# Sbte/RAILS

Hardware: AMD Instinct MI355X
Metric: RAILS iterations/sec (+ A*V SpMM HBM GB/s in roofline), m=1M rows/GPU, k=128, fp64 (higher is better)
Workload: dtype f64

## Files before the change

include/rails_hip.h:

```cpp
#ifndef RAILS_HIP_H
#define RAILS_HIP_H

#include <stddef.h>
#include <stdint.h>

#ifdef __cplusplus
extern "C" {
#endif

#define RAILS_OK 0
#define RAILS_EINVAL -1
#define RAILS_EHIP -2
#define RAILS_ENOMEM -3
#define RAILS_ELAPACK -4
#define RAILS_ECOMM -5
#define RAILS_ENODEV -6

typedef struct rails_ctx rails_ctx;
typedef struct rails_csr rails_csr;
typedef struct rails_panel rails_panel;

const char *rails_last_error(void);
const char *rails_version(void);

// ... 114 lines not shown
int rails_orthogonalize(rails_ctx *ctx, rails_panel *V, int k_old, int w, int method, int *used);
int rails_orthogonalize_deflated(rails_ctx *ctx, rails_panel *V, int k_old, int w, const rails_panel *N, int nc0, int q, int method, int *used);

int rails_resid_lanczos(rails_ctx *ctx, const rails_panel *AV, int avc0, const rails_panel *MV, int mvc0, int k,
                        const double *T_host, int ldt, const rails_panel *B, int bc0, int p, int L,
                        double *H_host, int ldh, int *steps);

int rails_lanczos_start(rails_ctx *ctx, const rails_panel *AV, int avc0, const rails_panel *MV, int mvc0, int k,
                        const rails_panel *B, int bc0, int p, double *sums_host);

int rails_lanczos_vectors(rails_ctx *ctx, const double *S_host, int lds, int w, rails_panel *Out, int oc0);
int rails_lanczos_release(rails_ctx *ctx);

int rails_ctx_reserve_staging(rails_ctx *ctx, size_t bytes);
int rails_timer_start(rails_ctx *ctx);
int rails_timer_stop(rails_ctx *ctx, double *ms);


void rails_sb03md(char dico, char job, char fact, char trans, int n, double *A, int lda, double *X, int ldx,
                  double *scale, int *info);
void rails_sb03md_counts(long *smith, long *schur);
void rails_sb03md_adi_counts(long *extended, long *fresh);
void rails_sb03md_set_pause(int calls);
void rails_dsyev(char jobz, char uplo, int n, double *a, int lda, double *w, int *info);
void rails_dsteqr(char compz, int n, double *d, double *e, double *z, int ldz, double *work, int *info);
void rails_dgemm(char transa, char transb, int m, int n, int k, double alpha, const double *A, int lda, const double *B,
                 int ldb, double beta, double *C, int ldc);
void rails_dtrsm(char side, char uplo, char transa, char diag, int m, int n, double alpha, const double *A, int lda, double *B, int ldb);
void rails_dpotrf(char uplo, int n, double *a, int lda, int *info);
void rails_dpstrf(char uplo, int n, double *a, int lda, int *piv, int *rank, double tol, int *info);
void rails_range_basis(int m, int n, double *a, int lda, double tol, double *q, int ldq, int *rank, int *info);
int rails_host_lapack_init(const char *path);
const char *rails_host_lapack_path(void);

#ifdef __cplusplus
}
#endif
#endif
```

rails_amd/_lib.py:

```python
import ctypes as C
import os

_HERE = os.path.dirname(os.path.abspath(__file__))
LIB_PATH = os.path.join(_HERE, "lib", "librails_hip.so")

_dp = C.POINTER(C.c_double)
_ip = C.POINTER(C.c_int)
_i64p = C.POINTER(C.c_int64)
_i32p = C.POINTER(C.c_int32)
_vp = C.c_void_p

ALLREDUCE_FN = C.CFUNCTYPE(C.c_int, C.c_void_p, C.c_void_p, C.c_size_t, C.c_void_p)
HALO_FN = C.CFUNCTYPE(C.c_int, C.c_void_p, C.c_void_p, C.c_void_p, C.c_int, C.c_void_p)
APPLY_FN = C.CFUNCTYPE(C.c_int, C.c_void_p, C.c_int, C.c_void_p, C.c_int, C.c_int, C.c_void_p, C.c_int)

SIGNATURES = {
    "rails_last_error": (C.c_char_p, []),
    "rails_version": (C.c_char_p, []),
    "rails_ctx_create": (C.c_int, [C.c_int, _vp, C.POINTER(_vp)]),
    "rails_ctx_destroy": (C.c_int, [_vp]),
    "rails_ctx_sync": (C.c_int, [_vp]),
    "rails_ctx_stream": (_vp, [_vp]),
    "rails_ctx_set_meter": (C.c_int, [_vp, C.c_int]),
    "rails_ctx_enable_library_gemm": (C.c_int, [_vp]),
# ... 55 lines not shown
    "rails_lu_solve": (C.c_int, [_vp, _vp, C.c_int, _vp, C.c_int, C.c_int, _vp, C.c_int]),
    "rails_lu_stats": (C.c_int, [_vp, _i64p, C.c_int]),
    "rails_csr_create_lu": (C.c_int, [_vp, _vp, C.POINTER(_vp)]),
    "rails_panel_random": (C.c_int, [_vp, _vp, C.c_int, C.c_int]),
    "rails_gram": (C.c_int, [_vp, _vp, C.c_int, C.c_int, _vp, C.c_int, C.c_int, _dp, C.c_int]),
    "rails_panel_gemm": (C.c_int, [_vp, C.c_double, _vp, C.c_int, C.c_int, _dp, C.c_int, C.c_int, C.c_double, _vp, C.c_int]),
    "rails_panel_gemm_wide": (C.c_int, [_vp, C.c_double, _vp, C.c_int, C.c_int, _dp, C.c_int, C.c_int, C.c_double, _vp, C.c_int]),
    "rails_orthogonalize": (C.c_int, [_vp, _vp, C.c_int, C.c_int, C.c_int, _ip]),
    "rails_orthogonalize_deflated": (C.c_int, [_vp, _vp, C.c_int, C.c_int, _vp, C.c_int, C.c_int, C.c_int, _ip]),
    "rails_resid_lanczos": (C.c_int, [_vp, _vp, C.c_int, _vp, C.c_int, C.c_int, _dp, C.c_int, _vp, C.c_int, C.c_int, C.c_int,
                                      _dp, C.c_int, _ip]),
    "rails_lanczos_start": (C.c_int, [_vp, _vp, C.c_int, _vp, C.c_int, C.c_int, _vp, C.c_int, C.c_int, _dp]),
    "rails_lanczos_vectors": (C.c_int, [_vp, _dp, C.c_int, C.c_int, _vp, C.c_int]),
    "rails_lanczos_release": (C.c_int, [_vp]),
    "rails_timer_start": (C.c_int, [_vp]),
    "rails_timer_stop": (C.c_int, [_vp, _dp]),
    "rails_sb03md": (None, [C.c_char, C.c_char, C.c_char, C.c_char, C.c_int, _dp, C.c_int, _dp, C.c_int, _dp, _ip]),
    "rails_dsyev": (None, [C.c_char, C.c_char, C.c_int, _dp, C.c_int, _dp, _ip]),
    "rails_dsteqr": (None, [C.c_char, C.c_int, _dp, _dp, _dp, C.c_int, _dp, _ip]),
    "rails_ctx_reserve_staging": (C.c_int, [_vp, C.c_size_t]),
    "rails_sb03md_set_pause": (None, [C.c_int]),
    "rails_sb03md_counts": (None, [C.POINTER(C.c_long), C.POINTER(C.c_long)]),
    "rails_sb03md_adi_counts": (None, [C.POINTER(C.c_long), C.POINTER(C.c_long)]),
    "rails_dtrsm": (None, [C.c_char, C.c_char, C.c_char, C.c_char, C.c_int, C.c_int, C.c_double, _dp, C.c_int, _dp, C.c_int]),
    "rails_dgemm": (None, [C.c_char, C.c_char, C.c_int, C.c_int, C.c_int, C.c_double, _dp, C.c_int, _dp, C.c_int, C.c_double, _dp, C.c_int]),
    "rails_dpotrf": (None, [C.c_char, C.c_int, _dp, C.c_int, _ip]),
    "rails_dpstrf": (None, [C.c_char, C.c_int, _dp, C.c_int, _ip, _ip, C.c_double, _ip]),
    "rails_range_basis": (None, [C.c_int, C.c_int, _dp, C.c_int, C.c_double, _dp, C.c_int, _ip, _ip]),
    "rails_host_lapack_init": (C.c_int, [C.c_char_p]),
    "rails_host_lapack_path": (C.c_char_p, []),
}

_lib = None


class RailsError(RuntimeError):
    pass


def load():
    global _lib
    if _lib is not None:
        return _lib
    if not os.path.exists(LIB_PATH):
        raise RailsError(
            "rails_amd: %s is missing -- build it with `python -c 'import __graft_entry__ as g; g.build()'` "
# ... 23 lines not shown
```

rails_amd/csrc/host_numerics.cpp:

```cpp
#include <dlfcn.h>

#include <algorithm>
#include <atomic>
#include <chrono>
#include <utility>
#include <cmath>
#include <cstdio>
#include <cstdlib>
#include <cstring>
#include <mutex>
#include <string>
#include <vector>

#include "rails_hip.h"

void rails_set_error(const char *fmt, ...);

namespace {

extern "C" {
typedef int (*lp_select2)(const double *, const double *);
typedef void (*lp_dsyev)(const char *, const char *, const int *, double *, const int *, double *, double *, const int *, int *);
typedef void (*lp_dsyevd)(const char *, const char *, const int *, double *, const int *, double *, double *, const int *, int *, const int *, int *);
typedef void (*lp_dsteqr)(const char *, const int *, double *, double *, double *, const int *, double *, int *);
// ... 327 lines not shown
    double wq = 0.0;
    int lwork = -1;
    g_lp.dgeqp3(&m, &n, a, &lda, jpvt.data(), tau.data(), &wq, &lwork, info);
    if (*info != 0) return;
    lwork = (int)wq + 1;
    std::vector<double> work((size_t)lwork);
    g_lp.dgeqp3(&m, &n, a, &lda, jpvt.data(), tau.data(), work.data(), &lwork, info);
    if (*info != 0) return;
    const double r11 = std::fabs(a[0]);
    int r = 0;
    while (r < kmin && std::fabs(a[r + (size_t)r * lda]) > tol * r11 && r11 > 0.0) ++r;
    *rank = r;
    if (r == 0) return;
    for (int j = 0; j < r; ++j)
        for (int i = 0; i < m; ++i) q[i + (size_t)j * ldq] = a[i + (size_t)j * lda];
    lwork = -1;
    g_lp.dorgqr(&m, &r, &r, q, &ldq, tau.data(), &wq, &lwork, info);
    if (*info != 0) return;
    lwork = (int)wq + 1;
    work.resize((size_t)lwork);
    g_lp.dorgqr(&m, &r, &r, q, &ldq, tau.data(), work.data(), &lwork, info);
}

static int &sb03md_smith_pause()
{
    static thread_local int pause = 0;
    return pause;
}
static int &sb03md_factored_pause()
{
    static thread_local int pause = 0;
    return pause;
}
extern "C" void rails_sb03md_set_pause(int calls) { sb03md_smith_pause() = sb03md_factored_pause() = calls > 0 ? calls : 0; }
static std::atomic<long> g_sb03md_smith{0}, g_sb03md_schur{0};
extern "C" void rails_sb03md_counts(long *smith, long *schur)
{
    if (smith) *smith = g_sb03md_smith.load();
    if (schur) *schur = g_sb03md_schur.load();
}

static bool smith_lyapunov(bool tr, int n, const double *A, int lda, double *X, int ldx)
{
    if (!g_lp.dgetrf || !g_lp.dgetrs) return false;
    const size_t nn = (size_t)n * n;
    std::vector<double> M(nn), S(nn), Ak(nn), Y(nn), T1(nn), T2(nn), C(nn);
    double trace = 0.0;
    for (int j = 0; j < n; ++j) {
        for (int i = 0; i < n; ++i) {
            M[i + (size_t)j * n] = tr ? A[i + (size_t)j * lda] : A[j + (size_t)i * lda];
            C[i + (size_t)j * n] = 0.5 * (X[i + (size_t)j * ldx] + X[j + (size_t)i * ldx]);
        }
        trace += A[j + (size_t)j * lda];
    }
    const double p = -trace / n;
    if (!(p > 0.0) || !std::isfinite(p)) return false;
    S = M;
// ... 34 lines not shown
    }
    if (!converged) return false;
    for (int j = 0; j < n; ++j)
        for (int i = 0; i < j; ++i) {
            const double v = 0.5 * (Y[i + (size_t)j * n] + Y[j + (size_t)i * n]);
            Y[i + (size_t)j * n] = v;
            Y[j + (size_t)i * n] = v;
        }
    gemm('N', 'N', n, n, n, M.data(), n, Y.data(), n, T1.data(), n);
    double r2 = 0.0;
    for (int j = 0; j < n; ++j)
        for (int i = 0; i < n; ++i) {
            const double r = T1[i + (size_t)j * n] + T1[j + (size_t)i * n] - C[i + (size_t)j * n];
            r2 += r * r;
        }
    if (!(std::sqrt(r2) <= 2e-15 * (2.0 * fro(M) * fro(Y) + fro(C)))) return false;
    for (int j = 0; j < n; ++j)
        for (int i = 0; i < n; ++i) X[i + (size_t)j * ldx] = Y[i + (size_t)j * n];
    return true;
}

struct AdiCache {
    int n = 0, L = 0;
    bool tr = false;
    double a = 0.0, b = 0.0;
    std::vector<double> M, shift;
    std::vector<std::vector<double>> LUs;
    std::vector<std::vector<int>> ips;
    std::vector<std::vector<double>> Inv;
};
static AdiCache &adi_cache()
{
    static thread_local AdiCache c;
    return c;
}
static std::atomic<long> g_adi_extended{0}, g_adi_fresh{0};
extern "C" void rails_sb03md_adi_counts(long *extended, long *fresh)
{
    if (extended) *extended = g_adi_extended.load();
    if (fresh) *fresh = g_adi_fresh.load();
}

static bool extend_lu(int n1, int n, const std::vector<double> &LU1, const std::vector<int> &ip1, std::vector<double> &S, std::vector<int> &ip)
{
    const int nb = n - n1, one = 1;
    const double d_one = 1.0, d_mone = -1.0;
// ... 45 lines not shown
        S = J1;
        return true;
    }
    const double d_one = 1.0, d_mone = -1.0, d_zero = 0.0;
    double *A12 = &S[(size_t)n1 * n], *A21 = &S[n1], *A22 = &S[n1 + (size_t)n1 * n];
    std::vector<double> E((size_t)n1 * nb), F((size_t)nb * n1), Cm((size_t)nb * nb), G((size_t)nb * n1);
    g_lp.dgemm("N", "N", &n1, &nb, &n1, &d_one, J1.data(), &n1, A12, &n, &d_zero, E.data(), &n1);
    g_lp.dgemm("N", "N", &nb, &n1, &n1, &d_one, A21, &n, J1.data(), &n1, &d_zero, F.data(), &nb);
    for (int j = 0; j < nb; ++j)
        for (int i = 0; i < nb; ++i) Cm[i + (size_t)j * nb] = A22[i + (size_t)j * n];
    g_lp.dgemm("N", "N", &nb, &nb, &n1, &d_mone, A21, &n, E.data(), &n1, &d_one, Cm.data(), &nb);
    if (!invert_dense(nb, Cm)) return false;
    g_lp.dgemm("N", "N", &nb, &n1, &nb, &d_one, Cm.data(), &nb, F.data(), &nb, &d_zero, G.data(), &nb);
    for (int j = 0; j < n1; ++j) memcpy(&S[(size_t)j * n], &J1[(size_t)j * n1], sizeof(double) * n1);
    g_lp.dgemm("N", "N", &n1, &n1, &nb, &d_one, E.data(), &n1, G.data(), &nb, &d_one, S.data(), &n);
    g_lp.dgemm("N", "N", &n1, &nb, &nb, &d_mone, E.data(), &n1, Cm.data(), &nb, &d_zero, A12, &n);
    for (int j = 0; j < n1; ++j)
        for (int i = 0; i < nb; ++i) A21[i + (size_t)j * n] = -G[i + (size_t)j * nb];
    for (int j = 0; j < nb; ++j)
        for (int i = 0; i < nb; ++i) A22[i + (size_t)j * n] = Cm[i + (size_t)j * nb];
    return true;
}

static bool adi_lyapunov_lowrank_once(bool tr, int n, const double *A, int lda, double *X, int ldx, bool *not_applicable, bool from_scratch, bool *inherited)
{
    *inherited = false;
    *not_applicable = false;
    if (!g_lp.dgetrf || !g_lp.dgetrs) return false;
    static const bool trace_lr = getenv("RAILS_SB03MD_TRACE") != nullptr;
    auto now = [] { return std::chrono::duration<double, std::milli>(std::chrono::steady_clock::now().time_since_epoch()).count(); };
    const double t_begin = now();
    double t_mark = t_begin, t_factor = 0, t_bounds = 0, t_lu = 0, t_terms = 0, t_form = 0;
    auto lap = [&](double &acc) {
        const double t = now();
        acc += t - t_mark;
        t_mark = t;
    };
    const size_t nn = (size_t)n * n;
    std::vector<double> C(nn), W(nn);
    double trc = 0.0, dmax = 0.0;
    for (int j = 0; j < n; ++j) {
        for (int i = 0; i < n; ++i) C[i + (size_t)j * n] = 0.5 * (X[i + (size_t)j * ldx] + X[j + (size_t)i * ldx]);
        trc += C[j + (size_t)j * n];
        dmax = std::max(dmax, std::fabs(C[j + (size_t)j * n]));
    }
    if (!(dmax > 0.0) || !std::isfinite(dmax)) return false;
    const double sign = trc >= 0.0 ? 1.0 : -1.0;
    for (size_t q = 0; q < nn; ++q) W[q] = sign * C[q];
    std::vector<int> piv(n);
    int rank = 0, info = 0;
    rails_dpstrf('U', n, W.data(), n, piv.data(), &rank, 1e-15 * dmax, &info);
    if (info < 0 || rank <= 0 || rank > n / 3) {
        *not_applicable = true;
        return false;
    }
    std::vector<double> F((size_t)n * rank, 0.0);
    for (int j = 0; j < n; ++j)
        for (int i = 0; i < rank && i <= j; ++i) F[piv[j] + (size_t)i * n] = W[i + (size_t)j * n];
    std::vector<double> M(nn);
    for (int j = 0; j < n; ++j)
        for (int i = 0; i < n; ++i) M[i + (size_t)j * n] = tr ? A[i + (size_t)j * lda] : A[j + (size_t)i * lda];
    lap(t_factor);
    const char N = 'N';
    const int one = 1;
    static const bool allow_inherit = !(getenv("RAILS_SB03MD_ADI_INHERIT") && atoi(getenv("RAILS_SB03MD_ADI_INHERIT")) == 0);
    AdiCache &cache = adi_cache();
    static const bool allow_explicit = !(getenv("RAILS_SB03MD_ADI_INVERSE") && atoi(getenv("RAILS_SB03MD_ADI_INVERSE")) == 0);
    const bool explicit_steps = allow_explicit && n >= 64;
    bool inherit = allow_inherit && !from_scratch && g_lp.dlaswp && g_lp.dtrsm && cache.n >= 32 && cache.tr == tr && n >= cache.n && n - cache.n <= 64 && cache.L >= 1 &&
                   (explicit_steps ? (int)cache.Inv.size() == cache.L : (int)cache.LUs.size() == cache.L);
    for (int j = 0; inherit && j < cache.n; ++j) inherit = memcmp(&M[(size_t)j * n], &cache.M[(size_t)j * cache.n], sizeof(double) * cache.n) == 0;
    double a = 0.0, b = 0.0;
    int L = 1;
    std::vector<double> shift;
    std::vector<std::vector<double>> LUs, Inv;
    std::vector<std::vector<int>> ips;
    std::vector<double> v(n), u(n);
    auto nrm = [&](std::vector<double> const &z) {
        double s2 = 0.0;
        for (int i = 0; i < n; ++i) s2 += z[i] * z[i];
        return std::sqrt(s2);
    };
    auto extent = [&](const std::vector<double> &LUp, const std::vector<int> &ipp, const std::vector<double> *InvP, double pshift, double *a_out, double *b_out) {
        for (int i = 0; i < n; ++i) v[i] = 1.0 + 0.37 * std::sin(1.0 + 2.3 * i);
        double bmax = 0.0, amin = 0.0;
        for (int it = 0; it < 6; ++it) {
            const double nv = nrm(v);
            for (int i = 0; i < n; ++i) v[i] /= nv;
            gemm('N', 'N', n, 1, n, M.data(), n, v.data(), n, u.data(), n);
            bmax = std::max(bmax, nrm(u));
            v = u;
        }
        for (int i = 0; i < n; ++i) v[i] = 1.0 + 0.37 * std::sin(1.0 + 2.3 * i);
        for (int it = 0; it < 6; ++it) {
            const double nv = nrm(v);
            for (int i = 0; i < n; ++i) v[i] /= nv;
            if (InvP) {
                gemm('N', 'N', n, 1, n, InvP->data(), n, v.data(), n, u.data(), n);
                v = u;
            } else {
                int inf = 0;
                g_lp.dgetrs(&N, &n, &one, LUp.data(), &n, ipp.data(), v.data(), &n, &inf);
                if (inf != 0) return false;
            }
            amin = nrm(v);
        }
        if (!(amin > 0.0) || !(bmax > 0.0) || !std::isfinite(amin) || !std::isfinite(bmax)) return false;
        const double lmin = 1.0 / amin - pshift;
        if (!(lmin > 0.0)) return false;
        *a_out = 0.8 * lmin, *b_out = 1.2 * bmax;
        if (!(*a_out < *b_out)) *a_out = 0.5 * *b_out;
        return true;
    };
    if (inherit) {
        a = cache.a, b = cache.b, L = cache.L, shift = cache.shift;
        LUs.assign(explicit_steps ? 0 : L, std::vector<double>());
        ips.assign(explicit_steps ? 0 : L, std::vector<int>());
        Inv.assign(explicit_steps ? L : 0, std::vector<double>());
        for (int i = 0; i < L && inherit; ++i) {
            std::vector<double> &S = explicit_steps ? Inv[i] : LUs[i];
            S = M;
            for (int j = 0; j < n; ++j) S[j + (size_t)j * n] -= shift[i];
            inherit = explicit_steps ? extend_inverse(cache.n, n, cache.Inv[i], S) : extend_lu(cache.n, n, cache.LUs[i], cache.ips[i], S, ips[i]);
        }
        lap(t_lu);
        double a_now = 0.0, b_now = 0.0;
        if (inherit && !((explicit_steps ? extent(Inv[0], std::vector<int>(), &Inv[0], shift[0], &a_now, &b_now) : extent(LUs[0], ips[0], nullptr, shift[0], &a_now, &b_now)) &&
                         a_now >= 0.8 * a && b_now <= 1.15 * b))
            inherit = false;
        lap(t_bounds);
    }
    if (!inherit) {
    std::vector<double> LU0 = M;
    std::vector<int> ip0(n);
    g_lp.dgetrf(&n, &n, LU0.data(), &n, ip0.data(), &info);
    if (info != 0) return false;
    if (!extent(LU0, ip0, nullptr, 0.0, &a, &b)) return false;
    lap(t_bounds);
    if (b / a > 1e5) return false;
    const double kappa = b / a, pi = 3.14159265358979323846;
    double best_cost = 1e300;
    for (int cand = 1; cand <= 8; cand *= 2) {
        double rho = cand == 1 ? (std::sqrt(kappa) - 1.0) / (std::sqrt(kappa) + 1.0) : std::min(0.999, 4.0 * std::exp(-pi * pi * cand / std::log(4.0 * kappa)));
        double sweeps = std::ceil(std::log(3e-9) / std::log(std::max(rho, 1e-300)));
        double cost = 4.0 * cand + cand * std::max(1.0, sweeps);
        if (cost < best_cost) best_cost = cost, L = cand;
    }
    shift.assign(1, std::sqrt(a * b));
    {
        std::vector<std::pair<double, double>> iv(1, std::make_pair(a, b));
        for (int l = L; l > 1; l /= 2) iv.push_back(std::make_pair(std::sqrt(iv.back().first * iv.back().second), 0.5 * (iv.back().first + iv.back().second)));
        shift.assign(1, std::sqrt(iv.back().first * iv.back().second));
        for (int lev = (int)iv.size() - 2; lev >= 0; --lev) {
            const double ab = iv[lev].first * iv[lev].second;
            std::vector<double> up;
            for (double x : shift) {
                const double d = std::sqrt(std::max(0.0, x * x - ab));
                up.push_back(x + d);
                up.push_back(x - d);
            }
            shift.swap(up);
        }
        std::sort(shift.begin(), shift.end());
    }
    LUs.assign(explicit_steps ? 0 : L, std::vector<double>());
    ips.assign(explicit_steps ? 0 : L, std::vector<int>(n));
    Inv.assign(explicit_steps ? L : 0, std::vector<double>());
    for (int i = 0; i < L; ++i) {
        std::vector<double> &S = explicit_steps ? Inv[i] : LUs[i];
        S = M;
        for (int j = 0; j < n; ++j) S[j + (size_t)j * n] -= shift[i];
        if (explicit_steps) {
            if (!invert_dense(n, S)) return false;
        } else {
            g_lp.dgetrf(&n, &n, S.data(), &n, ips[i].data(), &info);
            if (info != 0) return false;
        }
    }
    lap(t_lu);
    }
    (inherit ? g_adi_extended : g_adi_fresh)++;
    *inherited = inherit;
    lap(t_lu);
    const size_t blk = (size_t)n * rank;
    const int max_terms = std::max(64, 16 * L), max_cols = 8 * n;
    std::vector<double> Z, T(blk);
    Z.reserve(blk * 24);
    auto norm2 = [&](const double *z) {
        double s2 = 0.0;
        for (size_t q = 0; q < blk; ++q) s2 += z[q] * z[q];
        return s2;
    };
    std::vector<std::vector<double>> Sm(explicit_steps ? L : 0);
    for (int i = 0; i < (int)Sm.size(); ++i) {
        const double pj = shift[i], pp = shift[(i + L - 1) % L];
        const double f = std::sqrt(pj / pp), fg = f * (pj + pp);
        Sm[i].resize(nn);
        for (size_t q = 0; q < nn; ++q) Sm[i][q] = fg * Inv[i][q];
        for (int j = 0; j < n; ++j) Sm[i][j + (size_t)j * n] += f;
    }
    if (explicit_steps)
        gemm('N', 'N', n, rank, n, Inv[0].data(), n, F.data(), n, T.data(), n);
    else {
        T = F;
        g_lp.dgetrs(&N, &n, &rank, LUs[0].data(), &n, ips[0].data(), T.data(), &n, &info);
        if (info != 0) return false;
    }
    {
        const double f = std::sqrt(2.0 * shift[0]);
        for (size_t q = 0; q < blk; ++q) T[q] *= f;
    }
    Z.insert(Z.end(), T.begin(), T.end());
    double total = norm2(T.data()), cycle_start = total;
    bool converged = false;
    for (int j = 1; j < max_terms; ++j) {
        const int cur = j % L, prv = (j - 1) % L;
        const double pj = shift[cur], pp = shift[prv];
        const double *zp = Z.data() + (size_t)(j - 1) * blk;
        if (explicit_steps)
            gemm('N', 'N', n, rank, n, Sm[cur].data(), n, zp, n, T.data(), n);
        else {
            std::copy(zp, zp + blk, T.begin());
            g_lp.dgetrs(&N, &n, &rank, LUs[cur].data(), &n, ips[cur].data(), T.data(), &n, &info);
            if (info != 0) return false;
            const double f = std::sqrt(pj / pp), g = pj + pp;
            for (size_t q = 0; q < blk; ++q) T[q] = f * (zp[q] + g * T[q]);
        }
        const double n2 = norm2(T.data());
        if (!std::isfinite(n2) || n2 > 1e4 * total) return false;
        if ((int)((size_t)(j + 1) * rank) > max_cols) return false;
        Z.insert(Z.end(), T.begin(), T.end());
        total += n2;
        if (n2 <= 1e-17 * total) {
            converged = true;
            break;
        }
        if (cur == L - 1) {
            if (j >= 2 * L - 1 && n2 > 0.2 * cycle_start) {
                if (trace_lr) fprintf(stderr, "sb03md ADI: n %d, spectrum ~[%.3g, %.3g], %d shifts: term %d is %.2e of the same term one cycle earlier -- giving up\n", n, a, b, L, j, n2 / cycle_start);
                return false;
            }
            cycle_start = n2;
        }
    }
    lap(t_terms);
    if (trace_lr) fprintf(stderr, "sb03md ADI: n %d rank %d, spectrum ~[%.3g, %.3g], %d shifts, %d terms, converged %d\n", n, rank, a, b, L, (int)(Z.size() / blk), (int)converged);
    if (!converged) return false;
    const int cols = (int)(Z.size() / n);
    std::vector<double> Y(nn);
    if (g_lp.dsyrk) {
        const double one_d = 1.0, zero_d = 0.0;
        g_lp.dsyrk("U", "N", &n, &cols, &one_d, Z.data(), &n, &zero_d, Y.data(), &n);
        for (int j = 0; j < n; ++j)
            for (int i = 0; i < j; ++i) Y[j + (size_t)i * n] = Y[i + (size_t)j * n];
    } else {
        gemm('N', 'T', n, n, cols, Z.data(), n, Z.data(), n, Y.data(), n);
        for (int j = 0; j < n; ++j)
            for (int i = 0; i < j; ++i) {
                const double vv = 0.5 * (Y[i + (size_t)j * n] + Y[j + (size_t)i * n]);
                Y[i + (size_t)j * n] = vv;
                Y[j + (size_t)i * n] = vv;
            }
    }
    for (size_t q = 0; q < nn; ++q) Y[q] *= -sign;
    gemm('N', 'N', n, n, n, M.data(), n, Y.data(), n, W.data(), n);
    double r2 = 0.0, m2 = 0.0, y2 = 0.0, c2 = 0.0;
    for (int j = 0; j < n; ++j)
        for (int i = 0; i < n; ++i) {
            const double r = W[i + (size_t)j * n] + W[j + (size_t)i * n] - C[i + (size_t)j * n];
            r2 += r * r;
            m2 += M[i + (size_t)j * n] * M[i + (size_t)j * n];
            y2 += Y[i + (size_t)j * n] * Y[i + (size_t)j * n];
            c2 += C[i + (size_t)j * n] * C[i + (size_t)j * n];
        }
    lap(t_form);
    if (trace_lr)
        fprintf(stderr, "sb03md ADI: residual %.2e of %.2e allowed; ms: factor C %.2f, bounds %.2f, %d LU %.2f, terms %.2f, X = ZZ' + check %.2f, total %.2f\n", std::sqrt(r2),
                2e-15 * (2.0 * std::sqrt(m2 * y2) + std::sqrt(c2)), t_factor, t_bounds, L, t_lu, t_terms, t_form, now() - t_begin);
    if (!(std::sqrt(r2) <= 2e-15 * (2.0 * std::sqrt(m2 * y2) + std::sqrt(c2)))) return false;
    for (int j = 0; j < n; ++j)
        for (int i = 0; i < n; ++i) X[i + (size_t)j * ldx] = Y[i + (size_t)j * n];
    cache.n = n, cache.L = L, cache.tr = tr, cache.a = a, cache.b = b;
    cache.M.swap(M);
    cache.shift.swap(shift);
    cache.LUs.swap(LUs);
    cache.ips.swap(ips);
    cache.Inv.swap(Inv);
    return true;
}

static bool adi_lyapunov_lowrank(bool tr, int n, const double *A, int lda, double *X, int ldx, bool *not_applicable)
{
    bool inherited = false;
    if (adi_lyapunov_lowrank_once(tr, n, A, lda, X, ldx, not_applicable, false, &inherited)) return true;
    if (!inherited || *not_applicable) return false;
    return adi_lyapunov_lowrank_once(tr, n, A, lda, X, ldx, not_applicable, true, &inherited);
}

extern "C" void rails_sb03md(char dico, char job, char fact, char trans, int n, double *A, int lda, double *X, int ldx, double *scale,
                             int *info)
{
    *info = 0;
    if (n < 1) {
        fprintf(stderr, "rails_sb03md: n < 1 is not supported\n");
        return;
    }
    if ((dico != 'C' && dico != 'c') || (job != 'X' && job != 'x') || (fact != 'N' && fact != 'n')) {
        fprintf(stderr, "rails_sb03md: only DICO='C', JOB='X', FACT='N' is supported\n");
        *info = -1;
        return;
    }
    if (rails_host_lapack_init(nullptr) != RAILS_OK) {
        *info = -100;
        return;
    }
    if (!all_finite(n, n, A, lda) || !all_finite(n, n, X, ldx)) {
        fprintf(stderr, "rails_sb03md: A or C holds NaN or Inf entries\n");
        *info = n + 2;
        return;
    }
    const bool tr = (trans == 'T' || trans == 't' || trans == 'C' || trans == 'c');
    static const bool use_symmetric = [] {
        const char *e = getenv("RAILS_SB03MD_SYMMETRIC");
        return e ? atoi(e) != 0 : true;
    }();
    if (use_symmetric && n >= 8) {
        double amax = 0.0, asym = 0.0;
        for (int j = 0; j < n; ++j)
            for (int i = 0; i < j; ++i) {
                const double a = A[i + (size_t)j * lda], b = A[j + (size_t)i * lda];
                amax = std::max(amax, std::max(std::fabs(a), std::fabs(b)));
                asym = std::max(asym, std::fabs(a - b));
            }
        for (int i = 0; i < n; ++i) amax = std::max(amax, std::fabs(A[i + (size_t)i * lda]));
        if (amax > 0.0 && asym <= 1e-13 * amax) {
            std::vector<double> Q((size_t)n * n), lam(n), F((size_t)n * n), W((size_t)n * n);
            for (int j = 0; j < n; ++j)
                for (int i = 0; i < n; ++i) Q[i + (size_t)j * n] = 0.5 * (A[i + (size_t)j * lda] + A[j + (size_t)i * lda]);
            int sinfo = 0;
            if (g_lp.dsyevd) {
                int lwork = -1, liwork = -1, iq = 0;
                double wq = 0.0;
                g_lp.dsyevd("V", "U", &n, Q.data(), &n, lam.data(), &wq, &lwork, &iq, &liwork, &sinfo);
                lwork = (int)wq + 1;
// ... 8 lines not shown
            }
            if (sinfo == 0) {
                gemm('T', 'N', n, n, n, Q.data(), n, X, ldx, W.data(), n);
                gemm('N', 'N', n, n, n, W.data(), n, Q.data(), n, F.data(), n);
                bool singular = false;
                for (int j = 0; j < n && !singular; ++j)
                    for (int i = 0; i < n; ++i) {
                        const double den = lam[i] + lam[j];
                        if (!(std::fabs(den) > 1e-300)) {
                            singular = true;
                            break;
                        }
                        F[i + (size_t)j * n] /= den;
                    }
                if (!singular) {
                    gemm('N', 'N', n, n, n, Q.data(), n, F.data(), n, W.data(), n);
                    gemm('N', 'T', n, n, n, W.data(), n, Q.data(), n, F.data(), n);
                    for (int j = 0; j < n; ++j)
                        for (int i = 0; i < n; ++i) {
                            X[i + (size_t)j * ldx] = F[i + (size_t)j * n];
                            A[i + (size_t)j * lda] = (i == j) ? lam[i] : 0.0;
                        }
                    *scale = 1.0;
                    return;
                }
            }
        }
    }
    static const bool use_smith = [] {
        const char *e = getenv("RAILS_SB03MD_SMITH");
        return e ? atoi(e) != 0 : true;
    }();
    int &smith_pause = sb03md_smith_pause();
    int &lowrank_pause = sb03md_factored_pause();
    bool adi_na = false;
    if (use_smith && n >= 32) {
        if (smith_pause > 0)
            --smith_pause;
        else if ((lowrank_pause > 0 ? (--lowrank_pause, false) : (adi_lyapunov_lowrank(tr, n, A, lda, X, ldx, &adi_na) || (lowrank_pause = adi_na ? 0 : 30, false))) ||
                 smith_lyapunov(tr, n, A, lda, X, ldx)) {
            g_sb03md_smith++;
            *scale = 1.0;
            return;
        } else
            smith_pause = 30;
    }
    g_sb03md_schur++;
    std::vector<double> U((size_t)n * n), wr(n), wi(n), F((size_t)n * n), W((size_t)n * n);
    int sdim = 0, lwork = -1, linfo = 0;
    double wq = 0.0;
    g_lp.dgees("V", "N", nullptr, &n, A, &lda, &sdim, wr.data(), wi.data(), U.data(), &n, &wq, &lwork, nullptr, &linfo);
    lwork = std::max((int)wq, 3 * n);
    std::vector<double> work((size_t)lwork);
    g_lp.dgees("V", "N", nullptr, &n, A, &lda, &sdim, wr.data(), wi.data(), U.data(), &n, work.data(), &lwork, nullptr, &linfo);
    if (linfo != 0) {
        *info = linfo > n ? n : linfo;
        return;
    }
    gemm('T', 'N', n, n, n, U.data(), n, X, ldx, W.data(), n);
    gemm('N', 'N', n, n, n, W.data(), n, U.data(), n, F.data(), n);
    int isgn = 1, tinfo = 0;
    static const bool use_blocked = [] {
        const char *e = getenv("RAILS_SB03MD_BLOCKED");
        return e ? atoi(e) != 0 : true;
    }();
    bool done = false;
    if (g_lp.dtrsyl3 && use_blocked && n >= 64) {
        int liwork = -1, ldswork = -1, iq = 0, qinfo = 0;
        double sq[2] = {0.0, 0.0};
// ... 20 lines not shown
```

Before: 225.3.

## Restructure Lyapunov ADI solver with staged inheritance, reshifting, and adaptive backoff

Reworks the host-side low-rank ADI Lyapunov solver into a staged loop: inherited shifts, then re-shifting from freshly measured spectral bounds, then a from-scratch setup. An inherited attempt gives up early once it exceeds the previous call's term count. The fixed 30-call pause after failure becomes an exponential backoff capped at 32, and the ADI cache is cleared when the solver falls back. It also adds a per-call ring-buffer log of route, terms and time. The aim is to cut wasted ADI and Schur work in the small dense Lyapunov solves done each RAILS iteration, at the cost of more complex control flow and a small logging overhead on every call.

After: 221.2. -1.8%, worse.

```diff
diff --git a/include/rails_hip.h b/include/rails_hip.h
--- a/include/rails_hip.h
+++ b/include/rails_hip.h
@@ -160,6 +160,14 @@
 void rails_sb03md_counts(long *smith, long *schur);
 void rails_sb03md_adi_counts(long *extended, long *fresh);
 void rails_sb03md_set_pause(int calls);
+#define RAILS_SB03MD_ROUTE_SYMMETRIC 1
+#define RAILS_SB03MD_ROUTE_ADI_INHERITED 2
+#define RAILS_SB03MD_ROUTE_ADI_RESHIFTED 3
+#define RAILS_SB03MD_ROUTE_ADI_SCRATCH 4
+#define RAILS_SB03MD_ROUTE_SMITH 5
+#define RAILS_SB03MD_ROUTE_SCHUR 6
+int rails_sb03md_call_log(int max, int *n, int *route, int *terms, int *repeated, double *ms);
+void rails_sb03md_call_log_clear(void);
 void rails_dsyev(char jobz, char uplo, int n, double *a, int lda, double *w, int *info);
 void rails_dsteqr(char compz, int n, double *d, double *e, double *z, int ldz, double *work, int *info);
 void rails_dgemm(char transa, char transb, int m, int n, int k, double alpha, const double *A, int lda, const double *B,
diff --git a/rails_amd/_lib.py b/rails_amd/_lib.py
--- a/rails_amd/_lib.py
+++ b/rails_amd/_lib.py
@@ -101,6 +101,8 @@
     "rails_sb03md_set_pause": (None, [C.c_int]),
     "rails_sb03md_counts": (None, [C.POINTER(C.c_long), C.POINTER(C.c_long)]),
     "rails_sb03md_adi_counts": (None, [C.POINTER(C.c_long), C.POINTER(C.c_long)]),
+    "rails_sb03md_call_log": (C.c_int, [C.c_int, _ip, _ip, _ip, _ip, _dp]),
+    "rails_sb03md_call_log_clear": (None, []),
     "rails_dtrsm": (None, [C.c_char, C.c_char, C.c_char, C.c_char, C.c_int, C.c_int, C.c_double, _dp, C.c_int, _dp, C.c_int]),
     "rails_dgemm": (None, [C.c_char, C.c_char, C.c_int, C.c_int, C.c_int, C.c_double, _dp, C.c_int, _dp, C.c_int, C.c_double, _dp, C.c_int]),
     "rails_dpotrf": (None, [C.c_char, C.c_int, _dp, C.c_int, _ip]),
diff --git a/rails_amd/csrc/host_numerics.cpp b/rails_amd/csrc/host_numerics.cpp
--- a/rails_amd/csrc/host_numerics.cpp
+++ b/rails_amd/csrc/host_numerics.cpp
@@ -373,17 +373,66 @@
     g_lp.dorgqr(&m, &r, &r, q, &ldq, tau.data(), work.data(), &lwork, info);
 }
 
-static int &sb03md_smith_pause()
-{
-    static thread_local int pause = 0;
-    return pause;
-}
-static int &sb03md_factored_pause()
-{
-    static thread_local int pause = 0;
-    return pause;
-}
-extern "C" void rails_sb03md_set_pause(int calls) { sb03md_smith_pause() = sb03md_factored_pause() = calls > 0 ? calls : 0; }
+struct Sb03mdRest {
+    int rest = 0;
+    int pause = 0;
+    bool resting()
+    {
+        if (rest <= 0) return false;
+        --rest;
+        return true;
+    }
+    void failed() { rest = pause = pause > 0 ? std::min(2 * pause, 32) : 1; }
+    void succeeded() { pause = 0; }
+};
+static Sb03mdRest &sb03md_iterative_rest()
+{
+    static thread_local Sb03mdRest r;
+    return r;
+}
+static Sb03mdRest &sb03md_factored_rest()
+{
+    static thread_local Sb03mdRest r;
+    return r;
+}
+extern "C" void rails_sb03md_set_pause(int calls)
+{
+    Sb03mdRest forced;
+    forced.rest = calls > 0 ? calls : 0;
+    sb03md_iterative_rest() = sb03md_factored_rest() = forced;
+}
+
+struct Sb03mdCall {
+    int n, route, terms, repeated;
+    double ms;
+};
+struct Sb03mdLog {
+    static const int size = 256;
+    Sb03mdCall ring[size];
+    long count = 0;
+};
+static Sb03mdLog &sb03md_log()
+{
+    static thread_local Sb03mdLog log;
+    return log;
+}
+static double sb03md_now_ms() { return std::chrono::duration<double, std::milli>(std::chrono::steady_clock::now().time_since_epoch()).count(); }
+extern "C" int rails_sb03md_call_log(int max, int *n, int *route, int *terms, int *repeated, double *ms)
+{
+    const Sb03mdLog &log = sb03md_log();
+    const long held = std::min<long>(log.count, Sb03mdLog::size);
+    const int out = (int)std::min<long>(held, max > 0 ? max : 0);
+    for (int i = 0; i < out; ++i) {
+        const Sb03mdCall &c = log.ring[(log.count - out + i) % Sb03mdLog::size];
+        if (n) n[i] = c.n;
+        if (route) route[i] = c.route;
+        if (terms) terms[i] = c.terms;
+        if (repeated) repeated[i] = c.repeated;
+        if (ms) ms[i] = c.ms;
+    }
+    return out;
+}
+extern "C" void rails_sb03md_call_log_clear(void) { sb03md_log().count = 0; }
 static std::atomic<long> g_sb03md_smith{0}, g_sb03md_schur{0};
 extern "C" void rails_sb03md_counts(long *smith, long *schur)
 {
@@ -464,6 +513,7 @@
 
 struct AdiCache {
     int n = 0, L = 0;
+    int terms = 0;
     bool tr = false;
     double a = 0.0, b = 0.0;
     std::vector<double> M, shift;
@@ -555,17 +605,21 @@
     return true;
 }
 
-static bool adi_lyapunov_lowrank_once(bool tr, int n, const double *A, int lda, double *X, int ldx, bool *not_applicable, bool from_scratch, bool *inherited)
-{
-    *inherited = false;
+struct AdiOutcome {
+    int route = 0;
+    int terms = 0;
+    int wasted = 0;
+};
+
+static bool adi_lyapunov_lowrank(bool tr, int n, const double *A, int lda, double *X, int ldx, bool *not_applicable, AdiOutcome *outcome)
+{
     *not_applicable = false;
     if (!g_lp.dgetrf || !g_lp.dgetrs) return false;
     static const bool trace_lr = getenv("RAILS_SB03MD_TRACE") != nullptr;
-    auto now = [] { return std::chrono::duration<double, std::milli>(std::chrono::steady_clock::now().time_since_epoch()).count(); };
-    const double t_begin = now();
+    const double t_begin = sb03md_now_ms();
     double t_mark = t_begin, t_factor = 0, t_bounds = 0, t_lu = 0, t_terms = 0, t_form = 0;
     auto lap = [&](double &acc) {
-        const double t = now();
+        const double t = sb03md_now_ms();
         acc += t - t_mark;
         t_mark = t;
     };
@@ -600,7 +654,7 @@
     AdiCache &cache = adi_cache();
     static const bool allow_explicit = !(getenv("RAILS_SB03MD_ADI_INVERSE") && atoi(getenv("RAILS_SB03MD_ADI_INVERSE")) == 0);
     const bool explicit_steps = allow_explicit && n >= 64;
-    bool inherit = allow_inherit && !from_scratch && g_lp.dlaswp && g_lp.dtrsm && cache.n >= 32 && cache.tr == tr && n >= cache.n && n - cache.n <= 64 && cache.L >= 1 &&
+    bool inherit = allow_inherit && g_lp.dlaswp && g_lp.dtrsm && cache.n >= 32 && cache.tr == tr && n >= cache.n && n - cache.n <= 64 && cache.L >= 1 &&
                    (explicit_steps ? (int)cache.Inv.size() == cache.L : (int)cache.LUs.size() == cache.L);
     for (int j = 0; inherit && j < cache.n; ++j) inherit = memcmp(&M[(size_t)j * n], &cache.M[(size_t)j * cache.n], sizeof(double) * cache.n) == 0;
     double a = 0.0, b = 0.0;
@@ -614,10 +668,10 @@
         for (int i = 0; i < n; ++i) s2 += z[i] * z[i];
         return std::sqrt(s2);
     };
-    auto extent = [&](const std::vector<double> &LUp, const std::vector<int> &ipp, const std::vector<double> *InvP, double pshift, double *a_out, double *b_out) {
+    auto extent = [&](const std::vector<double> &LUp, const std::vector<int> &ipp, const std::vector<double> *InvP, double pshift, int steps, double *a_out, double *b_out) {
         for (int i = 0; i < n; ++i) v[i] = 1.0 + 0.37 * std::sin(1.0 + 2.3 * i);
         double bmax = 0.0, amin = 0.0;
-        for (int it = 0; it < 6; ++it) {
+        for (int it = 0; it < steps; ++it) {
             const double nv = nrm(v);
             for (int i = 0; i < n; ++i) v[i] /= nv;
             gemm('N', 'N', n, 1, n, M.data(), n, v.data(), n, u.data(), n);
@@ -625,7 +679,7 @@
             v = u;
         }
         for (int i = 0; i < n; ++i) v[i] = 1.0 + 0.37 * std::sin(1.0 + 2.3 * i);
-        for (int it = 0; it < 6; ++it) {
+        for (int it = 0; it < steps; ++it) {
             const double nv = nrm(v);
             for (int i = 0; i < n; ++i) v[i] /= nv;
             if (InvP) {
@@ -645,42 +699,15 @@
         if (!(*a_out < *b_out)) *a_out = 0.5 * *b_out;
         return true;
     };
-    if (inherit) {
-        a = cache.a, b = cache.b, L = cache.L, shift = cache.shift;
-        LUs.assign(explicit_steps ? 0 : L, std::vector<double>());
-        ips.assign(explicit_steps ? 0 : L, std::vector<int>());
-        Inv.assign(explicit_steps ? L : 0, std::vector<double>());
-        for (int i = 0; i < L && inherit; ++i) {
-            std::vector<double> &S = explicit_steps ? Inv[i] : LUs[i];
-            S = M;
-            for (int j = 0; j < n; ++j) S[j + (size_t)j * n] -= shift[i];
-            inherit = explicit_steps ? extend_inverse(cache.n, n, cache.Inv[i], S) : extend_lu(cache.n, n, cache.LUs[i], cache.ips[i], S, ips[i]);
-        }
-        lap(t_lu);
-        double a_now = 0.0, b_now = 0.0;
-        if (inherit && !((explicit_steps ? extent(Inv[0], std::vector<int>(), &Inv[0], shift[0], &a_now, &b_now) : extent(LUs[0], ips[0], nullptr, shift[0], &a_now, &b_now)) &&
-                         a_now >= 0.8 * a && b_now <= 1.15 * b))
-            inherit = false;
-        lap(t_bounds);
-    }
-    if (!inherit) {
-    std::vector<double> LU0 = M;
-    std::vector<int> ip0(n);
-    g_lp.dgetrf(&n, &n, LU0.data(), &n, ip0.data(), &info);
-    if (info != 0) return false;
-    if (!extent(LU0, ip0, nullptr, 0.0, &a, &b)) return false;
-    lap(t_bounds);
-    if (b / a > 1e5) return false;
-    const double kappa = b / a, pi = 3.14159265358979323846;
-    double best_cost = 1e300;
-    for (int cand = 1; cand <= 8; cand *= 2) {
-        double rho = cand == 1 ? (std::sqrt(kappa) - 1.0) / (std::sqrt(kappa) + 1.0) : std::min(0.999, 4.0 * std::exp(-pi * pi * cand / std::log(4.0 * kappa)));
-        double sweeps = std::ceil(std::log(3e-9) / std::log(std::max(rho, 1e-300)));
-        double cost = 4.0 * cand + cand * std::max(1.0, sweeps);
-        if (cost < best_cost) best_cost = cost, L = cand;
-    }
-    shift.assign(1, std::sqrt(a * b));
-    {
+    auto wachspress = [&]() {
+        const double kappa = b / a, pi = 3.14159265358979323846;
+        double best_cost = 1e300;
+        for (int cand = 1; cand <= 8; cand *= 2) {
+            double rho = cand == 1 ? (std::sqrt(kappa) - 1.0) / (std::sqrt(kappa) + 1.0) : std::min(0.999, 4.0 * std::exp(-pi * pi * cand / std::log(4.0 * kappa)));
+            double sweeps = std::ceil(std::log(3e-9) / std::log(std::max(rho, 1e-300)));
+            double cost = 4.0 * cand + cand * std::max(1.0, sweeps);
+            if (cost < best_cost) best_cost = cost, L = cand;
+        }
         std::vector<std::pair<double, double>> iv(1, std::make_pair(a, b));
         for (int l = L; l > 1; l /= 2) iv.push_back(std::make_pair(std::sqrt(iv.back().first * iv.back().second), 0.5 * (iv.back().first + iv.back().second)));
         shift.assign(1, std::sqrt(iv.back().first * iv.back().second));
@@ -695,125 +722,206 @@
             shift.swap(up);
         }
         std::sort(shift.begin(), shift.end());
-    }
-    LUs.assign(explicit_steps ? 0 : L, std::vector<double>());
-    ips.assign(explicit_steps ? 0 : L, std::vector<int>(n));
-    Inv.assign(explicit_steps ? L : 0, std::vector<double>());
-    for (int i = 0; i < L; ++i) {
+    };
+    auto prepare = [&]() {
+        LUs.assign(explicit_steps ? 0 : L, std::vector<double>());
+        ips.assign(explicit_steps ? 0 : L, std::vector<int>(n));
+        Inv.assign(explicit_steps ? L : 0, std::vector<double>());
+        for (int i = 0; i < L; ++i) {
+            std::vector<double> &S = explicit_steps ? Inv[i] : LUs[i];
+            S = M;
+            for (int j = 0; j < n; ++j) S[j + (size_t)j * n] -= shift[i];
+            if (explicit_steps) {
+                if (!invert_dense(n, S)) return false;
+            } else {
+                g_lp.dgetrf(&n, &n, S.data(), &n, ips[i].data(), &info);
+                if (info != 0) return false;
+            }
+        }
+        return true;
+    };
+    auto extend = [&](int i) {
         std::vector<double> &S = explicit_steps ? Inv[i] : LUs[i];
         S = M;
         for (int j = 0; j < n; ++j) S[j + (size_t)j * n] -= shift[i];
-        if (explicit_steps) {
-            if (!invert_dense(n, S)) return false;
-        } else {
-            g_lp.dgetrf(&n, &n, S.data(), &n, ips[i].data(), &info);
-            if (info != 0) return false;
-        }
-    }
-    lap(t_lu);
-    }
-    (inherit ? g_adi_extended : g_adi_fresh)++;
-    *inherited = inherit;
-    lap(t_lu);
+        return explicit_steps ? extend_inverse(cache.n, n, cache.Inv[i], S) : extend_lu(cache.n, n, cache.LUs[i], cache.ips[i], S, ips[i]);
+    };
     const size_t blk = (size_t)n * rank;
-    const int max_terms = std::max(64, 16 * L), max_cols = 8 * n;
-    std::vector<double> Z, T(blk);
-    Z.reserve(blk * 24);
+    const int max_cols = 8 * n;
+    std::vector<double> Z, T(blk), Y(nn);
     auto norm2 = [&](const double *z) {
         double s2 = 0.0;
         for (size_t q = 0; q < blk; ++q) s2 += z[q] * z[q];
         return s2;
     };
-    std::vector<std::vector<double>> Sm(explicit_steps ? L : 0);
-    for (int i = 0; i < (int)Sm.size(); ++i) {
-        const double pj = shift[i], pp = shift[(i + L - 1) % L];
-        const double f = std::sqrt(pj / pp), fg = f * (pj + pp);
-        Sm[i].resize(nn);
-        for (size_t q = 0; q < nn; ++q) Sm[i][q] = fg * Inv[i][q];
-        for (int j = 0; j < n; ++j) Sm[i][j + (size_t)j * n] += f;
-    }
-    if (explicit_steps)
-        gemm('N', 'N', n, rank, n, Inv[0].data(), n, F.data(), n, T.data(), n);
-    else {
-        T = F;
-        g_lp.dgetrs(&N, &n, &rank, LUs[0].data(), &n, ips[0].data(), T.data(), &n, &info);
-        if (info != 0) return false;
-    }
-    {
-        const double f = std::sqrt(2.0 * shift[0]);
-        for (size_t q = 0; q < blk; ++q) T[q] *= f;
-    }
-    Z.insert(Z.end(), T.begin(), T.end());
-    double total = norm2(T.data()), cycle_start = total;
-    bool converged = false;
-    for (int j = 1; j < max_terms; ++j) {
-        const int cur = j % L, prv = (j - 1) % L;
-        const double pj = shift[cur], pp = shift[prv];
-        const double *zp = Z.data() + (size_t)(j - 1) * blk;
+    auto iterate = [&](int give_up_after) {
+        const int max_terms = std::max(64, 16 * L);
+        Z.clear();
+        Z.reserve(blk * 24);
+        std::vector<std::vector<double>> Sm(explicit_steps ? L : 0);
+        for (int i = 0; i < (int)Sm.size(); ++i) {
+            const double pj = shift[i], pp = shift[(i + L - 1) % L];
+            const double f = std::sqrt(pj / pp), fg = f * (pj + pp);
+            Sm[i].resize(nn);
+            for (size_t q = 0; q < nn; ++q) Sm[i][q] = fg * Inv[i][q];
+            for (int j = 0; j < n; ++j) Sm[i][j + (size_t)j * n] += f;
+        }
         if (explicit_steps)
-            gemm('N', 'N', n, rank, n, Sm[cur].data(), n, zp, n, T.data(), n);
+            gemm('N', 'N', n, rank, n, Inv[0].data(), n, F.data(), n, T.data(), n);
         else {
-            std::copy(zp, zp + blk, T.begin());
-            g_lp.dgetrs(&N, &n, &rank, LUs[cur].data(), &n, ips[cur].data(), T.data(), &n, &info);
+            T = F;
+            g_lp.dgetrs(&N, &n, &rank, LUs[0].data(), &n, ips[0].data(), T.data(), &n, &info);
             if (info != 0) return false;
-            const double f = std::sqrt(pj / pp), g = pj + pp;
-            for (size_t q = 0; q < blk; ++q) T[q] = f * (zp[q] + g * T[q]);
-        }
-        const double n2 = norm2(T.data());
-        if (!std::isfinite(n2) || n2 > 1e4 * total) return false;
-        if ((int)((size_t)(j + 1) * rank) > max_cols) return false;
+        }
+        {
+            const double f = std::sqrt(2.0 * shift[0]);
+            for (size_t q = 0; q < blk; ++q) T[q] *= f;
+        }
         Z.insert(Z.end(), T.begin(), T.end());
-        total += n2;
-        if (n2 <= 1e-17 * total) {
-            converged = true;
+        double total = norm2(T.data()), cycle_start = total;
+        for (int j = 1; j < max_terms; ++j) {
+            const int cur = j % L, prv = (j - 1) % L;
+            const double pj = shift[cur], pp = shift[prv];
+            const double *zp = Z.data() + (size_t)(j - 1) * blk;
+            if (explicit_steps)
+                gemm('N', 'N', n, rank, n, Sm[cur].data(), n, zp, n, T.data(), n);
+            else {
+                std::copy(zp, zp + blk, T.begin());
+                g_lp.dgetrs(&N, &n, &rank, LUs[cur].data(), &n, ips[cur].data(), T.data(), &n, &info);
+                if (info != 0) return false;
+                const double f = std::sqrt(pj / pp), g = pj + pp;
+                for (size_t q = 0; q < blk; ++q) T[q] = f * (zp[q] + g * T[q]);
+            }
+            const double n2 = norm2(T.data());
+            if (!std::isfinite(n2) || n2 > 1e4 * total) return false;
+            if ((int)((size_t)(j + 1) * rank) > max_cols) return false;
+            Z.insert(Z.end(), T.begin(), T.end());
+            total += n2;
+            if (n2 <= 1e-17 * total) return true;
+            if (j + 1 > give_up_after) {
+                if (trace_lr) fprintf(stderr, "sb03md ADI: n %d, inherited shifts: %d terms and not converged (the call before took %d) -- giving the attempt up\n", n, j + 1, cache.terms);
+                return false;
+            }
+            if (cur == L - 1) {
+                if (j >= 2 * L - 1 && n2 > 0.2 * cycle_start) {
+                    if (trace_lr) fprintf(stderr, "sb03md ADI: n %d, spectrum ~[%.3g, %.3g], %d shifts: term %d is %.2e of the same term one cycle earlier -- giving up\n", n, a, b, L, j, n2 / cycle_start);
+                    return false;
+                }
+                cycle_start = n2;
+            }
+        }
+        return false;
+    };
+    auto accept = [&]() {
+        const int cols = (int)(Z.size() / n);
+        if (g_lp.dsyrk) {
+            const double one_d = 1.0, zero_d = 0.0;
+            g_lp.dsyrk("U", "N", &n, &cols, &one_d, Z.data(), &n, &zero_d, Y.data(), &n);
+            for (int j = 0; j < n; ++j)
+                for (int i = 0; i < j; ++i) Y[j + (size_t)i * n] = Y[i + (size_t)j * n];
+        } else {
+            gemm('N', 'T', n, n, cols, Z.data(), n, Z.data(), n, Y.data(), n);
+            for (int j = 0; j < n; ++j)
+                for (int i = 0; i < j; ++i) {
+                    const double vv = 0.5 * (Y[i + (size_t)j * n] + Y[j + (size_t)i * n]);
+                    Y[i + (size_t)j * n] = vv;
+                    Y[j + (size_t)i * n] = vv;
+                }
+        }
+        for (size_t q = 0; q < nn; ++q) Y[q] *= -sign;
+        gemm('N', 'N', n, n, n, M.data(), n, Y.data(), n, W.data(), n);
+        double r2 = 0.0, m2 = 0.0, y2 = 0.0, c2 = 0.0;
+        for (int j = 0; j < n; ++j)
+            for (int i = 0; i < n; ++i) {
+                const double r = W[i + (size_t)j * n] + W[j + (size_t)i * n] - C[i + (size_t)j * n];
+                r2 += r * r;
+                m2 += M[i + (size_t)j * n] * M[i + (size_t)j * n];
+                y2 += Y[i + (size_t)j * n] * Y[i + (size_t)j * n];
+                c2 += C[i + (size_t)j * n] * C[i + (size_t)j * n];
+            }
+        lap(t_form);
+        if (trace_lr)
+            fprintf(stderr, "sb03md ADI: residual %.2e of %.2e allowed; ms: factor C %.2f, bounds %.2f, %d LU %.2f, terms %.2f, X = ZZ' + check %.2f, total %.2f\n", std::sqrt(r2),
+                    2e-15 * (2.0 * std::sqrt(m2 * y2) + std::sqrt(c2)), t_factor, t_bounds, L, t_lu, t_terms, t_form, sb03md_now_ms() - t_begin);
+        return std::sqrt(r2) <= 2e-15 * (2.0 * std::sqrt(m2 * y2) + std::sqrt(c2));
+    };
+
+    int stage = inherit ? RAILS_SB03MD_ROUTE_ADI_INHERITED : RAILS_SB03MD_ROUTE_ADI_SCRATCH;
+    double a_now = 0.0, b_now = 0.0;
+    auto measure = [&](int steps) {
+        return explicit_steps ? extent(Inv[0], std::vector<int>(), &Inv[0], shift[0], steps, &a_now, &b_now) : extent(LUs[0], ips[0], nullptr, shift[0], steps, &a_now, &b_now);
+    };
+    for (;;) {
+        int give_up_after = 1 << 30;
+        if (stage == RAILS_SB03MD_ROUTE_ADI_INHERITED) {
+            a = cache.a, b = cache.b, L = cache.L, shift = cache.shift;
+            LUs.assign(explicit_steps ? 0 : L, std::vector<double>());
+            ips.assign(explicit_steps ? 0 : L, std::vector<int>());
+            Inv.assign(explicit_steps ? L : 0, std::vector<double>());
+            if (!extend(0)) {
+                stage = RAILS_SB03MD_ROUTE_ADI_SCRATCH;
+                continue;
+            }
+            lap(t_lu);
+            const bool covered = measure(6) && a_now >= 0.8 * a && b_now <= 1.15 * b;
+            lap(t_bounds);
+            if (!covered) {
+                stage = measure(30) ? RAILS_SB03MD_ROUTE_ADI_RESHIFTED : RAILS_SB03MD_ROUTE_ADI_SCRATCH;
+                lap(t_bounds);
+                continue;
+            }
+            bool extended = true;
+            for (int i = 1; i < L && extended; ++i) extended = extend(i);
+            lap(t_lu);
+            if (!extended) {
+                stage = RAILS_SB03MD_ROUTE_ADI_SCRATCH;
+                continue;
+            }
+            if (cache.terms > 0) give_up_after = cache.terms + L;
+        } else {
+            if (stage == RAILS_SB03MD_ROUTE_ADI_RESHIFTED) {
+                a = a_now, b = b_now;
+                if (b / a > 1e5) {
+                    stage = RAILS_SB03MD_ROUTE_ADI_SCRATCH;
+                    continue;
+                }
+            } else {
+                std::vector<double> LU0 = M;
+                std::vector<int> ip0(n);
+                g_lp.dgetrf(&n, &n, LU0.data(), &n, ip0.data(), &info);
+                if (info != 0) return false;
+                if (!extent(LU0, ip0, nullptr, 0.0, 6, &a, &b)) return false;
+                lap(t_bounds);
+                if (b / a > 1e5) return false;
+            }
+            wachspress();
+            if (!prepare()) return false;
+            lap(t_lu);
+        }
+        (stage == RAILS_SB03MD_ROUTE_ADI_INHERITED ? g_adi_extended : g_adi_fresh)++;
+        const bool converged = iterate(give_up_after);
+        const int terms = (int)(Z.size() / blk);
+        lap(t_terms);
+        if (trace_lr)
+            fprintf(stderr, "sb03md ADI (%s): n %d rank %d, spectrum ~[%.3g, %.3g], %d shifts, %d terms, converged %d\n",
+                    stage == RAILS_SB03MD_ROUTE_ADI_INHERITED ? "inherited" : stage == RAILS_SB03MD_ROUTE_ADI_RESHIFTED ? "re-shifted" : "from scratch", n, rank, a, b, L, terms, (int)converged);
+        if (converged && accept()) {
+            outcome->route = stage;
+            outcome->terms = terms;
             break;
         }
-        if (cur == L - 1) {
-            if (j >= 2 * L - 1 && n2 > 0.2 * cycle_start) {
-                if (trace_lr) fprintf(stderr, "sb03md ADI: n %d, spectrum ~[%.3g, %.3g], %d shifts: term %d is %.2e of the same term one cycle earlier -- giving up\n", n, a, b, L, j, n2 / cycle_start);
-                return false;
-            }
-            cycle_start = n2;
-        }
-    }
-    lap(t_terms);
-    if (trace_lr) fprintf(stderr, "sb03md ADI: n %d rank %d, spectrum ~[%.3g, %.3g], %d shifts, %d terms, converged %d\n", n, rank, a, b, L, (int)(Z.size() / blk), (int)converged);
-    if (!converged) return false;
-    const int cols = (int)(Z.size() / n);
-    std::vector<double> Y(nn);
-    if (g_lp.dsyrk) {
-        const double one_d = 1.0, zero_d = 0.0;
-        g_lp.dsyrk("U", "N", &n, &cols, &one_d, Z.data(), &n, &zero_d, Y.data(), &n);
-        for (int j = 0; j < n; ++j)
-            for (int i = 0; i < j; ++i) Y[j + (size_t)i * n] = Y[i + (size_t)j * n];
-    } else {
-        gemm('N', 'T', n, n, cols, Z.data(), n, Z.data(), n, Y.data(), n);
-        for (int j = 0; j < n; ++j)
-            for (int i = 0; i < j; ++i) {
-                const double vv = 0.5 * (Y[i + (size_t)j * n] + Y[j + (size_t)i * n]);
-                Y[i + (size_t)j * n] = vv;
-                Y[j + (size_t)i * n] = vv;
-            }
-    }
-    for (size_t q = 0; q < nn; ++q) Y[q] *= -sign;
-    gemm('N', 'N', n, n, n, M.data(), n, Y.data(), n, W.data(), n);
-    double r2 = 0.0, m2 = 0.0, y2 = 0.0, c2 = 0.0;
-    for (int j = 0; j < n; ++j)
-        for (int i = 0; i < n; ++i) {
-            const double r = W[i + (size_t)j * n] + W[j + (size_t)i * n] - C[i + (size_t)j * n];
-            r2 += r * r;
-            m2 += M[i + (size_t)j * n] * M[i + (size_t)j * n];
-            y2 += Y[i + (size_t)j * n] * Y[i + (size_t)j * n];
-            c2 += C[i + (size_t)j * n] * C[i + (size_t)j * n];
-        }
-    lap(t_form);
-    if (trace_lr)
-        fprintf(stderr, "sb03md ADI: residual %.2e of %.2e allowed; ms: factor C %.2f, bounds %.2f, %d LU %.2f, terms %.2f, X = ZZ' + check %.2f, total %.2f\n", std::sqrt(r2),
-                2e-15 * (2.0 * std::sqrt(m2 * y2) + std::sqrt(c2)), t_factor, t_bounds, L, t_lu, t_terms, t_form, now() - t_begin);
-    if (!(std::sqrt(r2) <= 2e-15 * (2.0 * std::sqrt(m2 * y2) + std::sqrt(c2)))) return false;
+        outcome->wasted += terms;
+        if (stage == RAILS_SB03MD_ROUTE_ADI_INHERITED)
+            stage = measure(30) ? RAILS_SB03MD_ROUTE_ADI_RESHIFTED : RAILS_SB03MD_ROUTE_ADI_SCRATCH;
+        else if (stage == RAILS_SB03MD_ROUTE_ADI_RESHIFTED)
+            stage = RAILS_SB03MD_ROUTE_ADI_SCRATCH;
+        else
+            return false;
+        lap(t_bounds);
+    }
     for (int j = 0; j < n; ++j)
         for (int i = 0; i < n; ++i) X[i + (size_t)j * ldx] = Y[i + (size_t)j * n];
-    cache.n = n, cache.L = L, cache.tr = tr, cache.a = a, cache.b = b;
+    cache.n = n, cache.L = L, cache.tr = tr, cache.a = a, cache.b = b, cache.terms = outcome->terms;
     cache.M.swap(M);
     cache.shift.swap(shift);
     cache.LUs.swap(LUs);
@@ -822,14 +930,6 @@
     return true;
 }
 
-static bool adi_lyapunov_lowrank(bool tr, int n, const double *A, int lda, double *X, int ldx, bool *not_applicable)
-{
-    bool inherited = false;
-    if (adi_lyapunov_lowrank_once(tr, n, A, lda, X, ldx, not_applicable, false, &inherited)) return true;
-    if (!inherited || *not_applicable) return false;
-    return adi_lyapunov_lowrank_once(tr, n, A, lda, X, ldx, not_applicable, true, &inherited);
-}
-
 extern "C" void rails_sb03md(char dico, char job, char fact, char trans, int n, double *A, int lda, double *X, int ldx, double *scale,
                              int *info)
 {
@@ -853,6 +953,17 @@
         return;
     }
     const bool tr = (trans == 'T' || trans == 't' || trans == 'C' || trans == 'c');
+    struct Record {
+        Sb03mdCall call;
+        const double t0 = sb03md_now_ms();
+        ~Record()
+        {
+            Sb03mdLog &log = sb03md_log();
+            call.ms = sb03md_now_ms() - t0;
+            log.ring[log.count++ % Sb03mdLog::size] = call;
+        }
+    } record;
+    record.call = Sb03mdCall{n, RAILS_SB03MD_ROUTE_SCHUR, 0, 0, 0.0};
     static const bool use_symmetric = [] {
         const char *e = getenv("RAILS_SB03MD_SYMMETRIC");
         return e ? atoi(e) != 0 : true;
@@ -907,6 +1018,7 @@
                             A[i + (size_t)j * lda] = (i == j) ? lam[i] : 0.0;
                         }
                     *scale = 1.0;
+                    record.call.route = RAILS_SB03MD_ROUTE_SYMMETRIC;
                     return;
                 }
             }
@@ -916,20 +1028,30 @@
         const char *e = getenv("RAILS_SB03MD_SMITH");
         return e ? atoi(e) != 0 : true;
     }();
-    int &smith_pause = sb03md_smith_pause();
-    int &lowrank_pause = sb03md_factored_pause();
-    bool adi_na = false;
+    Sb03mdRest &iterative = sb03md_iterative_rest();
+    Sb03mdRest &factored = sb03md_factored_rest();
     if (use_smith && n >= 32) {
-        if (smith_pause > 0)
-            --smith_pause;
-        else if ((lowrank_pause > 0 ? (--lowrank_pause, false) : (adi_lyapunov_lowrank(tr, n, A, lda, X, ldx, &adi_na) || (lowrank_pause = adi_na ? 0 : 30, false))) ||
-                 smith_lyapunov(tr, n, A, lda, X, ldx)) {
-            g_sb03md_smith++;
-            *scale = 1.0;
-            return;
+        const bool factored_rests = factored.resting();
+        if (!iterative.resting()) {
+            bool adi_na = false;
+            AdiOutcome adi;
+            const bool by_adi = !factored_rests && adi_lyapunov_lowrank(tr, n, A, lda, X, ldx, &adi_na, &adi);
+            if (!factored_rests && !adi_na) by_adi ? factored.succeeded() : factored.failed();
+            record.call.repeated = adi.wasted;
+            if (!by_adi && !adi_na) adi_cache().n = 0;
+            if (by_adi || smith_lyapunov(tr, n, A, lda, X, ldx)) {
+                iterative.succeeded();
+                record.call.route = by_adi ? adi.route : RAILS_SB03MD_ROUTE_SMITH;
+                record.call.terms = adi.terms;
+                g_sb03md_smith++;
+                *scale = 1.0;
+                return;
+            }
+            iterative.failed();
         } else
-            smith_pause = 30;
-    }
+            adi_cache().n = 0;
+    }
+    record.call.route = RAILS_SB03MD_ROUTE_SCHUR;
     g_sb03md_schur++;
     std::vector<double> U((size_t)n * n), wr(n), wi(n), F((size_t)n * n), W((size_t)n * n);
     int sdim = 0, lwork = -1, linfo = 0;
```
